# centreborelli/sat-bundleadjust

Measured on AMD Instinct MI355X. Metric: LM iters/sec at 200 cams x 1M pts x 10M obs (affine, R+T), higher is better.
Workload: dtype f64; 1 GPU; C4: 200 cams x 1000000 pts x 9998866 obs, affine, correction R+T, 1 fixed camera, seed 1; obs_per_rank0=9998866

## Files before the change

sat-bundleadjust_amd/csrc/satba_capi.hip:

```cpp
#include <hip/hip_runtime.h>

#include <algorithm>
#include <atomic>
#include <chrono>
#include <cmath>
#include <cstdarg>
#include <cstdio>
#include <cstdlib>
#include <cstring>
#include <new>
#include <string>
#include <thread>
#include <vector>

#include "../../include/satba.h"
#include "satba_chol.h"
#include "satba_kernels.h"
#include "satba_layout.h"
#include "satba_lm.h"
#include "satba_lmdev.h"
#include "satba_outliers.h"
#include "satba_triangulate.h"
#include "satba_rpcfit.h"
#include "satba_schur.h"
// ... 50 lines not shown
    long long K = 0, n_total = 0;
    int n_c = 0, n = 0, hdr = 0;
    int loss = 0;
    int camc_lds = 0, rpc_lds = 0;
    int cam_sums_lds = 1;
    int lin_rep_shift = 0;
    int deterministic = 0;
    double *d_fx = nullptr, *d_bbox = nullptr, *d_fxcost = nullptr, *d_fxcost_new = nullptr, *d_fxcost0 = nullptr;
    int *d_fxflag = nullptr, *d_fxe = nullptr;
    bool fxcost_valid = false, fxcost_new_valid = false, fxcost0_valid = false;
    bool decide_fused = false;
    double w_max = 1.0, n_max_cam = 1.0, fx_shrink = 1.0;
    int fx_fallbacks = 0;
    bool scales_by_tail = false;
    bool skip_lin_scales = false;
    const int* gate = nullptr;
    const double* Delta_dev = nullptr;
    const int* first_dev = nullptr;
    const double* coef_dev = nullptr;
    int fuse_prep = -1;
    bool prep_fused = false;
    const double* lam_force_dev = nullptr;
    const double* sub_args_dev = nullptr;
    struct LmDev* d_lm = nullptr;
    struct LmSummary* h_lm = nullptr;
    struct LmSummary* h_lm_dev = nullptr;
    long long lm_ticks_queued = 0;
    hipStream_t own_stream = nullptr;
    double f_scale = 1.0, lead = 1.0;
    hipStream_t stream = nullptr;
    Layout L;
    int unit_weights = 0;
    double *d_cam_static = nullptr, *d_rpc = nullptr;
    double *d_x = nullptr, *d_xnew = nullptr, *d_camc = nullptr, *d_camc_new = nullptr;
    double *d_scale_inv = nullptr, *d_g = nullptr, *d_gh = nullptr, *d_gn = nullptr, *d_q1 = nullptr, *d_wv = nullptr;
    double *d_U = nullptr, *d_gc = nullptr, *d_V = nullptr, *d_Vinv = nullptr, *d_PV = nullptr, *d_dc = nullptr, *d_dch = nullptr;
    double2 *d_f = nullptr, *d_ftmp = nullptr;
    bool f_valid = false;
    bool prof_lin = false;
    std::vector<hipEvent_t> prof_ev;
    size_t prof_used = 0;
    double* d_Jpm = nullptr;
    double *d_part = nullptr, *d_part3 = nullptr, *d_pair_part = nullptr;
    int2* d_items = nullptr;
    SchurItem* d_item_desc = nullptr;
    double2* d_W = nullptr;
    int2* d_items_w = nullptr;
    SchurItem* d_item_desc_w = nullptr;
    int n_item_blocks_w = 0;
    int2* d_items_merged = nullptr;
    SchurItem* d_item_desc_merged = nullptr;
    int n_item_blocks_merged = 0;
    int n_item_blocks = 0;
    int lin_grid = 0, cm_chunks = 1, cm_chunks_w = 1;
    double* d_red = nullptr;
    unsigned* d_red_cnt = nullptr;
    double* d_stage = nullptr;
    size_t stage_len = 0;
    int* d_fail = nullptr;
    double* d_dinv = nullptr;
    CholWork chol;
    bool scale_in_finish = false;
    bool s_scaled = false;
    double schur_lam = 0.0;
    const double* schur_lam_dev = nullptr;
    hipStream_t chol_stream = nullptr;
    hipEvent_t ev_fork = nullptr, ev_join = nullptr;
    int* d_arrive = nullptr;
    int* d_pair_cnt = nullptr;
    int* d_dg_cnt = nullptr;
    long long* d_ts = nullptr;
    int arrive_epoch = 0;
    bool decide2_fused = false;
    int msg_epoch = 0;
    double* msg_packed = nullptr;
    bool beside_last = false;
    bool beside_off = false;
    int beside_clean = 0;
    int beside_retry_after = 64;
    int beside_timeouts = 0;
    double* d_scal = nullptr;
    double* d_keep = nullptr;
    bool prepared = false;
    double *d_xb_own = nullptr, *d_xb = nullptr;
    long long xb_len = 0;
    double* h_pin = nullptr;
    bool dir_global = false;
    double* d_dir_tab = nullptr;
    void* h_stage = nullptr;
    size_t h_stage_len = 0;
    struct CopyLane { char* pin = nullptr; hipEvent_t ev[2] = {nullptr, nullptr}; };
    CopyLane lanes[8];
    hipStream_t copy_stream = nullptr;
    bool lanes_ready = false;
    double* d_err_keep = nullptr;
    hipEvent_t ev_err = nullptr;
    double* d_x0 = nullptr;
    bool linearized = false, have_step = false;
    double create_ms[8] = {0, 0, 0, 0, 0, 0, 0, 0};
    std::vector<void*> allocs;

    double* payload() const { return d_xb + hdr; }
    RedBuf red(int slot) const { return RedBuf{d_red + (size_t)slot * RED_MAX_NV * RED_MAX_GRID, d_red_cnt + slot}; }
};
enum { RB_RES = 0, RB_LIN = 1, RB_PREP = 2, RB_JVP = 3, RB_BS = 4, RB_SUB = 5, RB_TRIAL = 6, RB_MISC = 7 };

// ... 230 lines not shown
static int launch_linearize_kernel(satba_problem* p) {
    ObsArgs a = obs_args(p, false);
    a.sh = slice_split(p);
    a.rev = slice_rev(0);
    if (p->fuse_prep >= 0) {
        a.prep_scale = p->d_scale_inv; a.prep_gh = p->d_gh; a.prep_ghs = p->d_q1;
        a.prep_first = p->fuse_prep; a.prep_first_dev = p->first_dev;
    }
    const bool prof = p->prof_lin && p->prof_used + 2 <= 2 * 4096;
    if (prof) {
        while (p->prof_ev.size() < p->prof_used + 2) {
            hipEvent_t e;
            HIP_TRY(hipEventCreate(&e));
            p->prof_ev.push_back(e);
        }
        HIP_TRY(hipEventRecord(p->prof_ev[p->prof_used], p->stream));
    }
    SATBA_DISPATCH(p, TRY((launch_lin<MODEL, NP, CL, RL>(p, a))));
    if (prof) {
        HIP_TRY(hipEventRecord(p->prof_ev[p->prof_used + 1], p->stream));
        p->prof_used += 2;
    }
    return 0;
}

static int launch_cam_sums(satba_problem* p, double* U, double* gc) {
    ObsArgs a = obs_args(p, false);
    CamMajor cm = cam_major(p);
    SATBA_DISPATCH(p, hipLaunchKernelGGL((k_cam_sums<MODEL, NP>), dim3(p->M, p->cm_chunks), dim3(LINC_THREADS), 0, p->stream, a, cm, p->d_f, p->d_part3));
    HIP_TRY(hipGetLastError());
    const int total = p->M * cam_acc_len(p->NP);
    hipLaunchKernelGGL(k_cam_sums_finish, dim3((total + 255) / 256), dim3(256), 0, p->stream, p->M, p->NP, p->cm_chunks, p->d_part3, U, gc, p->gate);
    HIP_TRY(hipGetLastError());
    return 0;
}

static SchurArgs schur_args(const satba_problem* p) {
    SchurArgs s;
    s.PV = reinterpret_cast<const double2*>(p->d_PV);
    s.pair_ofs = p->L.pair_ofs; s.pair_pts = p->L.pair_pts; s.pair_pi = p->L.pair_pi; s.pair_pj = p->L.pair_pj;
    s.pair_ij = p->L.pair_ij; s.pair_part = p->d_pair_part; s.n_chunks = p->L.C; s.items = p->d_items; s.desc = p->d_item_desc;
    if (wmode(p) && p->L.wl_ready) {
        s.PV = p->d_W; s.wmode = 1; s.zero_fix = p->L.zero_fix; s.n_dg = p->L.n_dg;
        s.pair_rec = p->L.pair_rec; s.pair_kk = p->L.pair_kk; s.cm_rec = p->L.cm_rec; s.cm_sc = p->L.cm_sc; s.dg_part = p->d_part3;
        s.items = p->d_items_w; s.desc = p->d_item_desc_w;
    }
    return s;
}

template <int MODEL, int NP>
static int launch_schur(satba_problem* p, const ObsArgs& a, double* S, double* rhs) {
    CamMajor cm = cam_major(p);
    SchurArgs s = schur_args(p);
    const long long n_pairs = p->L.n_pairs;
    const bool pairs_run = n_pairs > 0 && p->L.E > 0;
    const bool dg_in_pairs = s.wmode && MODEL != RPC && pairs_run;
    int dchunks = (a.sc && MODEL != RPC) ? p->cm_chunks_w : p->cm_chunks;
    static const bool one_launch_env = !(getenv("SATBA_SCHUR_ONE_LAUNCH") && atoi(getenv("SATBA_SCHUR_ONE_LAUNCH")) == 0);
    const bool both = one_launch_env && !p->arrive_epoch && !dg_in_pairs && pairs_run;
    if (dg_in_pairs) dchunks = p->L.n_dg;
    else {
        if (s.wmode) cm.pt = p->L.cm_rec;
        s.diag_xcd = (dchunks % 8 == 0 && !getenv("SATBA_NO_DIAG_XCD")) ? 1 : 0;
        if (!both) hipLaunchKernelGGL((k_schur_diag<MODEL, NP>), dim3(p->M, dchunks), dim3(LINC_THREADS), 0, p->stream, a, cm, s, p->d_part3);
    }
    const int total = p->M * cam_acc_len(NP);
    const int nb_diag = (int)((std::max<long long>(8ll * total, p->hdr) + 255) / 256);
    auto finish = [&](int red_chunks, bool direct) {
        const long long outs = red_chunks > 1 ? n_pairs * NP * NP : 0;
        const bool scale = p->scale_in_finish && !direct && 1 + CH_MAX_STEPS <= nb_diag * 256;
        hipLaunchKernelGGL(k_schur_finish, dim3((unsigned)(nb_diag + (outs + 255) / 256)), dim3(256), 0, p->stream, p->M, NP, p->n_c, dchunks, p->d_part3,
                           p->schur_lam, p->schur_lam_dev, p->lead, p->d_gc, p->d_scale_inv, S, rhs, p->d_xb, (int)p->hdr, nb_diag, red_chunks,
                           p->L.pair_ij, p->d_pair_part, p->gate, scale ? p->d_dch : (double*)nullptr, scale ? p->d_fail : (int*)nullptr,
                           scale ? 1 + CH_MAX_STEPS : 0);
        p->s_scaled = scale;
    };
    if (p->arrive_epoch) {
        if (dg_in_pairs) {
            const int keep = dchunks;
            dchunks = 0;
            finish(1, true);
            dchunks = keep;
            s.dg_cnt = p->d_dg_cnt; s.dg_lam = p->schur_lam; s.dg_lam_dev = p->schur_lam_dev; s.dg_lead = p->lead; s.dg_gc = p->d_gc;
            s.dg_scale_inv = p->d_scale_inv; s.dg_rhs = rhs;
        } else finish(1, true);
        s.arrive = p->d_arrive; s.arrive_epoch = p->arrive_epoch; s.pair_cnt = p->d_pair_cnt; s.fail = p->d_fail;
    }
    int red_chunks = 1;
    if (n_pairs > 0 && p->L.E > 0) {
        const bool merged = a.unit && p->d_item_desc_merged;
        if (merged) { s.desc = p->d_item_desc_merged; s.items = p->d_items_merged; s.n_chunks = 1; }
        const dim3 igrid((unsigned)(merged ? p->n_item_blocks_merged : (s.wmode ? p->n_item_blocks_w : p->n_item_blocks)));
        if (both) {
            const int n_diag = p->M * dchunks, n_diag_pad = (n_diag + 7) & ~7;
            const dim3 bgrid(igrid.x + (unsigned)n_diag_pad);
            if (a.unit) hipLaunchKernelGGL((k_schur_both<MODEL, NP, true>), bgrid, dim3(256), 0, p->stream, a, cm, s, p->d_part3, S, n_diag, n_diag_pad, p->M, dchunks);
            else hipLaunchKernelGGL((k_schur_both<MODEL, NP, false>), bgrid, dim3(256), 0, p->stream, a, cm, s, p->d_part3, S, n_diag, n_diag_pad, p->M, dchunks);
        }
        else if (a.unit) hipLaunchKernelGGL((k_schur_pairs<MODEL, NP, true>), igrid, dim3(256), 0, p->stream, a, s, S);
        else hipLaunchKernelGGL((k_schur_pairs<MODEL, NP, false>), igrid, dim3(256), 0, p->stream, a, s, S);
        HIP_TRY(hipGetLastError());
        if (p->L.C > 1 && !merged) red_chunks = p->L.C;
        if (p->arrive_epoch && (a.unit ? red_chunks > 1 : false)) return fail(SATBA_E_STATE, "factorisation beside a unit-weight pair kernel with chunk partials");
    }
    if (!p->arrive_epoch) finish(red_chunks, n_pairs > 0 && p->L.E > 0 && red_chunks == 1);
    HIP_TRY(hipGetLastError());
    return 0;
}

static int launch_schur_kernel(satba_problem* p) {
    ObsArgs a = obs_args(p, false);
    double* S = p->payload();
    double* rhs = S + (size_t)p->n_c * p->n_c;
    SATBA_DISPATCH(p, TRY((launch_schur<MODEL, NP>(p, a, S, rhs))));
    return 0;
}

static int launch_backsub_kernel(satba_problem* p) {
    ObsArgs a = obs_args(p, false);
    a.sh = slice_split(p);
    a.rev = slice_rev(1);
    const int grid = slice_grid(p, BS_THREADS / 64, 2, a.sh);
    const size_t lds = p->model == AFFINE ? dir_table_bytes(p) : table_bytes(p);
    if (p->dir_global) {
        SATBA_DISPATCH(p, if constexpr (MODEL == AFFINE) {
            hipLaunchKernelGGL((k_affine_dir_tab<NP>), dim3(1), dim3(1024), 0, p->stream, a, p->d_dc, (const double*)nullptr, (const double*)nullptr);
            hipLaunchKernelGGL((k_backsub<MODEL, NP, CL, RL, true>), dim3(grid), dim3(BS_THREADS), 0, p->stream, a, p->d_dc, p->d_dch, p->lead,
                               p->d_Vinv, p->d_g, p->d_scale_inv, p->d_gh, p->d_gn, p->red(RB_BS), p->d_xb);
        });
    } else
    SATBA_DISPATCH(p, hipLaunchKernelGGL((k_backsub<MODEL, NP, CL, RL>), dim3(grid), dim3(BS_THREADS), lds, p->stream, a, p->d_dc, p->d_dch, p->lead,
                                         p->d_Vinv, p->d_g, p->d_scale_inv, p->d_gh, p->d_gn, p->red(RB_BS), p->d_xb));
    HIP_TRY(hipGetLastError());
    return 0;
}

static int launch_jvp(satba_problem* p, int nv, const double* q1, const double* q2, double* out, bool pre = false) {
    ObsArgs a = obs_args(p, false);
    a.sh = slice_split(p);
    a.rev = slice_rev(2);
    const int grid = slice_grid(p, JVP_THREADS / 64, 2, a.sh);
    const RedBuf rb = p->red(RB_JVP);
    if (p->dir_global && (nv == 2 || pre)) {
        SATBA_DISPATCH(p, if constexpr (MODEL == AFFINE) {
            hipLaunchKernelGGL((k_affine_dir_tab<NP>), dim3(1), dim3(1024), 0, p->stream, a, q1, nv == 2 ? q2 : nullptr, nv == 2 ? p->d_scale_inv : nullptr);
// ... 402 lines not shown
        TRY(dev_alloc(p, &p->d_cam_static, (size_t)p->M * p->c_p));
        if (p->model == RPC) TRY(dev_alloc(p, &p->d_rpc, (size_t)p->M * SATBA_RPC_TABLE_LEN));
        TRY(dev_alloc(p, &p->d_x, n)); TRY(dev_alloc(p, &p->d_xnew, n)); TRY(dev_alloc(p, &p->d_scale_inv, n));
        TRY(dev_alloc(p, &p->d_g, n)); TRY(dev_alloc(p, &p->d_gh, n)); TRY(dev_alloc(p, &p->d_gn, n));
        TRY(dev_alloc(p, &p->d_q1, n)); TRY(dev_alloc(p, &p->d_wv, n));
        TRY(dev_alloc(p, &p->d_camc, (size_t)p->M * CAMC)); TRY(dev_alloc(p, &p->d_camc_new, (size_t)p->M * CAMC));
        TRY(dev_alloc(p, &p->d_U, (size_t)p->M * p->NP * p->NP)); TRY(dev_alloc(p, &p->d_gc, p->n_c));
        TRY(dev_alloc(p, &p->d_V, (size_t)6 * p->N)); TRY(dev_alloc(p, &p->d_Vinv, (size_t)6 * p->N));
        TRY(dev_alloc(p, &p->d_PV, (size_t)PV_STRIDE * (p->N + 1)));
        HIP_TRY(hipMemset(p->d_PV + (size_t)PV_STRIDE * p->N, 0, sizeof(double) * PV_STRIDE));
        TRY(dev_alloc(p, &p->d_dc, p->n_c)); TRY(dev_alloc(p, &p->d_dch, p->n_c));
        const size_t Kz = (size_t)std::max<long long>(K, 1) + 64;
        TRY(dev_alloc(p, &p->d_f, Pz)); TRY(dev_alloc(p, &p->d_ftmp, Pz));
        if (p->model == RPC) TRY(dev_alloc(p, &p->d_Jpm, Kz * jrow_stride(p->NP)));
        TRY(dev_alloc(p, &p->d_fail, 1 + CH_MAX_STEPS));
        TRY(dev_alloc(p, &p->d_dinv, (size_t)((p->n_c + CH_NB - 1) / CH_NB) * CH_NB * CH_NB));
        {
            const size_t T = (size_t)(p->n_c + 63) / 64;
            TRY(dev_alloc(p, &p->chol.flags, T * T + 1)); TRY(dev_alloc(p, &p->chol.Linv, T * 4096 + 1)); TRY(dev_alloc(p, &p->chol.Cc, T * T * 64 + 1));
            TRY(dev_alloc(p, &p->chol.ctr, 4));
            HIP_TRY(hipMemset(p->chol.flags, 0, sizeof(int) * (T * T + 1)));
            HIP_TRY(hipMemset(p->chol.ctr, 0, sizeof(int) * 4));
        }
        TRY(dev_alloc(p, &p->d_scal, 8));
        TRY(dev_alloc(p, &p->d_fx, fx_scales_len(p->NP))); TRY(dev_alloc(p, &p->d_fxe, fx_exps_len(p->NP)));
        TRY(dev_alloc(p, &p->d_bbox, 6)); TRY(dev_alloc(p, &p->d_fxflag, 1));
        TRY(dev_alloc(p, &p->d_fxcost, 1)); TRY(dev_alloc(p, &p->d_fxcost_new, 1)); TRY(dev_alloc(p, &p->d_fxcost0, 1));
        HIP_TRY(hipMemset(p->d_bbox, 0, sizeof(double) * 6));
        HIP_TRY(hipMemset(p->d_fxflag, 0, sizeof(int)));
        if (const char* fs = getenv("SATBA_FX_SHRINK")) p->fx_shrink = atof(fs);
        TRY(dev_alloc(p, &p->d_lm, 1));
        HIP_TRY(hipMemset(p->d_lm, 0, sizeof(LmDev)));
        HIP_TRY(hipHostMalloc((void**)&p->h_lm, sizeof(LmSummary) + sizeof(LmDev), hipHostMallocMapped));
        memset(p->h_lm, 0, sizeof(LmSummary) + sizeof(LmDev));
        HIP_TRY(hipHostGetDevicePointer((void**)&p->h_lm_dev, p->h_lm, 0));
        TRY(dev_alloc(p, &p->d_keep, SATBA_KEEP_LEN));
        HIP_TRY(hipMemset(p->d_keep, 0, sizeof(double) * SATBA_KEEP_LEN));
        TRY(dev_alloc(p, &p->d_red, (size_t)RED_SLOTS * RED_MAX_NV * RED_MAX_GRID));
        TRY(dev_alloc(p, &p->d_red_cnt, RED_SLOTS));
        HIP_TRY(hipMemset(p->d_red_cnt, 0, sizeof(unsigned) * RED_SLOTS));
        p->lin_grid = lin_grid_for(p);
        TRY(dev_alloc(p, &p->d_part, (size_t)512 * p->M * cam_sum_len(p->NP)));
        {
            int chunks = 8;
            while (chunks < 64 && (long long)p->M * chunks < 512 && K / ((long long)p->M * (chunks + 8)) >= 4096) chunks += 8;
            while (chunks > 1 && K / ((long long)p->M * chunks) < 256) --chunks;
            int chunks_w = chunks;
            if (chunks >= 8) {
                chunks_w = std::min(64, 2 * chunks);
                while (chunks_w > chunks && K / ((long long)p->M * chunks_w) < 512) chunks_w -= 8;
            }
            if (const char* dc = getenv("SATBA_CM_CHUNKS")) chunks_w = chunks = std::max(1, std::min(256, atoi(dc)));
            p->cm_chunks = chunks; p->cm_chunks_w = chunks_w;
            TRY(dev_alloc(p, &p->d_part3, (size_t)p->M * std::max(64, std::max(chunks, chunks_w)) * (cam_acc_len(p->NP) + p->NP)));
        }
        if (p->L.C > 1) TRY(dev_alloc(p, &p->d_pair_part, (size_t)p->L.C * std::max<long long>(p->L.n_pairs, 1) * p->NP * p->NP));
        TRY(schur_item_table(p));
        p->stage_len = std::max<size_t>(std::max<size_t>(n, 2 * (size_t)K), (size_t)6 * p->N) + 16;
        TRY(dev_alloc(p, &p->d_stage, p->stage_len));
        p->xb_len = satba_exchange_len(p);
        TRY(dev_alloc(p, &p->d_xb_own, p->xb_len));
        p->d_xb = p->d_xb_own;
        HIP_TRY(hipHostMalloc((void**)&p->h_pin, sizeof(double) * (p->hdr + 64)));
        HIP_TRY(hipMemset(p->d_xb, 0, sizeof(double) * p->xb_len));
        HIP_TRY(hipMemset(p->d_scale_inv, 0, sizeof(double) * n));
        HIP_TRY(hipMemset(p->d_x, 0, sizeof(double) * n));
        HIP_TRY(hipMemset(p->d_xnew, 0, sizeof(double) * n));
        HIP_TRY(hipMemcpy(p->d_cam_static, d->cam_params, sizeof(double) * p->M * p->c_p, hipMemcpyHostToDevice));
        if (p->model == RPC)
            HIP_TRY(hipMemcpy(p->d_rpc, d->rpc_tables, sizeof(double) * p->M * SATBA_RPC_TABLE_LEN, hipMemcpyHostToDevice));
        return 0;
    }();
    if (rc) {
        satba_problem_destroy(p);
        return rc;
    }
    p->create_ms[4] = ms_since(t_create);
    *out = p;
    return 0;
}

void satba_problem_destroy(satba_problem* p) {
    if (!p) return;
    (void)hipSetDevice(p->device);
    (void)hipDeviceSynchronize();
#ifdef C3_STAMPS
    if (p->d_ts) {
        std::vector<long long> ts((size_t)20 * C3_TS);
        (void)hipMemcpy(ts.data(), p->d_ts, sizeof(long long) * ts.size(), hipMemcpyDeviceToHost);
        const int T = (p->n_c + 63) / 64;
        const long long t0 = ts[(size_t)T * C3_TS + 0];
        fprintf(stderr, "C3TS wait_begin 0 chain_start %.2f\n", (ts[(size_t)T * C3_TS + 1] - t0) * 0.01);
        for (int k = 0; k < T; ++k) {
            fprintf(stderr, "C3TS step %2d start %8.2f D_done %8.2f R %8.2f I %8.2f dnext %8.2f aux %8.2f nextD %8.2f | col arrived %8.2f handed %8.2f\n", k,
                    (ts[(size_t)k * C3_TS + 0] - t0) * 0.01, (ts[(size_t)k * C3_TS + 1] - t0) * 0.01, (ts[(size_t)k * C3_TS + 2] - t0) * 0.01,
                    (ts[(size_t)k * C3_TS + 3] - t0) * 0.01, (ts[(size_t)k * C3_TS + 4] - t0) * 0.01, (ts[(size_t)k * C3_TS + 5] - t0) * 0.01,
                    (ts[(size_t)k * C3_TS + 6] - t0) * 0.01, k >= 2 ? (ts[(size_t)T * C3_TS + k] - t0) * 0.01 : 0.0,
                    k >= 2 ? (ts[(size_t)(T + 1) * C3_TS + k] - t0) * 0.01 : 0.0);
        }
    }
#endif
    for (void* q : p->allocs) (void)hipFree(q);
    for (hipEvent_t e : p->prof_ev) (void)hipEventDestroy(e);
    if (p->h_pin) (void)hipHostFree(p->h_pin);
    if (p->h_stage) (void)hipHostFree(p->h_stage);
    for (auto& l : p->lanes) { if (l.pin) (void)hipHostFree(l.pin); for (hipEvent_t e : l.ev) if (e) (void)hipEventDestroy(e); }
    if (p->copy_stream) (void)hipStreamDestroy(p->copy_stream);
    if (p->ev_err) (void)hipEventDestroy(p->ev_err);
    if (p->h_lm) (void)hipHostFree(p->h_lm);
    if (p->own_stream) (void)hipStreamDestroy(p->own_stream);
    if (p->chol_stream) (void)hipStreamDestroy(p->chol_stream);
    if (p->ev_fork) (void)hipEventDestroy(p->ev_fork);
    if (p->ev_join) (void)hipEventDestroy(p->ev_join);
    delete p;
}

int satba_set_stream(satba_problem* p, void* hip_stream, int32_t use_own) {
    if (!p) return fail(SATBA_E_ARG, "null handle");
    HIP_TRY(hipSetDevice(p->device));
    HIP_TRY(hipStreamSynchronize(p->stream));
    p->stream = use_own ? p->own_stream : static_cast<hipStream_t>(hip_stream);
    return 0;
}

int64_t satba_header_len(const satba_problem* p) { return p ? p->hdr : 0; }

int64_t satba_exchange_len(const satba_problem* p) {
    if (!p) return 0;
    const long long lin = (long long)p->M * p->NP * p->NP + p->n_c;
    const long long sch = (long long)p->n_c * p->n_c + p->n_c;
    return p->hdr + (lin > sch ? lin : sch);
}

int satba_bind_exchange(satba_problem* p, double* device_ptr, int64_t len) {
    if (!p) return fail(SATBA_E_ARG, "null handle");
    if (!device_ptr) { p->d_xb = p->d_xb_own; return 0; }
    if (len < satba_exchange_len(p)) return fail(SATBA_E_ARG, "exchange buffer too small: %lld < %lld", (long long)len, (long long)satba_exchange_len(p));
    p->d_xb = device_ptr;
    return 0;
}

__global__ __launch_bounds__(256) void k_pack_lower(int n, int hdr, double* __restrict__ xb, double* __restrict__ packed, int unpack, int c_lo, int c_hi,
                                                    const int* gate) {
    SATBA_GATE(gate);
    const int j = blockIdx.x;
    if (j == n) {
        if (c_lo != 0) return;
        for (int i = threadIdx.x; i < hdr + n; i += 256) {
            double* a = i < hdr ? xb + i : xb + hdr + (size_t)n * n + (i - hdr);
            double* b = packed + i;
            if (unpack) __hip_atomic_store(a, __hip_atomic_load(b, __ATOMIC_RELAXED, __HIP_MEMORY_SCOPE_SYSTEM), __ATOMIC_RELAXED, __HIP_MEMORY_SCOPE_AGENT);
// ... 1289 lines not shown
```

sat-bundleadjust_amd/csrc/satba_schur.h:

```cpp
#pragma once
#include "satba_kernels.h"

namespace satba {

constexpr int PV_STRIDE = 16;
__device__ inline double schur_lambda(const double* __restrict__ hdr, double Delta, double lam_floor, double* __restrict__ keep, bool write) {
    const double gh_sq = hdr[1], jg_sq = hdr[2], xs_sq = hdr[3];
    if (!(Delta > 0.0)) {
        Delta = sqrt(xs_sq);
        if (Delta == 0.0) Delta = 1.0;
    }
    const double a = 0.5 * jg_sq, b = -gh_sq, ub = Delta / sqrt(gh_sq);
    double best = fmin(0.0, a * ub * ub + b * ub);
    if (a != 0.0) {
        const double ext = -0.5 * b / a;
        if (0.0 < ext && ext < ub) best = fmin(best, a * ext * ext + b * ext);
    }
    double lam = -best / (Delta * Delta);
    if (!(lam >= lam_floor)) lam = lam_floor;
    if (write) {
        keep[1] = fmax(keep[1], hdr[4]);
        keep[2] = gh_sq; keep[3] = jg_sq; keep[4] = xs_sq;
        keep[5] = lam;
        keep[6] = Delta;
// ... 63 lines not shown
#pragma unroll
        for (int k = 0; k < 8; ++k) {
            const int g = 64 * k + lane, r = g >> 3, q = g & 7;
            const double2 v = t[9 * r + (q < 6 ? q : 0)];
            const int at = w_fix[min(p0 + r, N - 1)];
            if (q < 6 && r < n_here) out[(size_t)at + q] = v;
        }
        return;
    }
    {
        double2* out = reinterpret_cast<double2*>(PV + PV_STRIDE * (size_t)p0);
#pragma unroll
        for (int k = 0; k < 8; ++k) {
            const int g = 64 * k + lane, r = g >> 3, q = g & 7;
            const double2 v = t[9 * r + (q < 6 ? q : 0)];
            if (q < 6 && r < n_here) out[g] = v;
        }
    }
}

struct SchurItem {
    long long lo, hi;
    int i, j;
    int pair, chunk;
};
struct SchurArgs {
    const double2* __restrict__ PV;
    const long long* __restrict__ pair_ofs;
    const int* __restrict__ pair_pts;
    const int* __restrict__ pair_pi;
    const int* __restrict__ pair_pj;
    const int2* __restrict__ pair_ij;
    double* __restrict__ pair_part;
    const int2* __restrict__ items;
    const struct SchurItem* __restrict__ desc;
    int n_chunks;
    int diag_xcd = 0;
    int wmode = 0, zero_fix = 0, n_dg = 1;
    const int* __restrict__ pair_rec = nullptr;
    const int* __restrict__ pair_kk = nullptr;
    const int* __restrict__ cm_rec = nullptr;
    const int* __restrict__ cm_sc = nullptr;
    double* __restrict__ dg_part = nullptr;
    int* dg_cnt = nullptr;
    double dg_lam = 0.0, dg_lead = 1.0;
    const double* dg_lam_dev = nullptr;
    const double* __restrict__ dg_gc = nullptr;
    const double* __restrict__ dg_scale_inv = nullptr;
    double* __restrict__ dg_rhs = nullptr;
    int* arrive = nullptr;
    int arrive_epoch = 0;
    int* pair_cnt = nullptr;
    int* fail = nullptr;
};
constexpr int SCHUR_ARRIVE_STRIDE = 32;

template <int N>
__device__ inline double wave_reduce_scatter(const double (&v)[N], int lane, int mask) {
    if constexpr (N == 1) {
        double t = v[0];
        for (int m = mask; m > 0; m >>= 1) t += __shfl_xor(t, m);
        return t;
    } else {
        constexpr int H = N / 2;
        const bool upper = (lane & mask) != 0;
        double w[H];
#pragma unroll
        for (int k = 0; k < H; ++k) {
            const double keep = upper ? v[k + H] : v[k];
            const double send = upper ? v[k] : v[k + H];
            w[k] = keep + __shfl_xor(send, mask);
        }
        return wave_reduce_scatter<H>(w, lane, mask >> 1);
    }
}
template <int N>
__device__ inline int rs_index(int lane) {
    int idx = 0, mask = 32;
    for (int h = N / 2; h >= 1; h >>= 1, mask >>= 1)
        if (lane & mask) idx += h;
    return idx;
}

__global__ void k_schur_item_desc(long long n_items, const int2* __restrict__ items, const int2* __restrict__ pair_ij,
                                  const long long* __restrict__ pair_ofs, int n_chunks, SchurItem* __restrict__ desc,
                                  const int* __restrict__ dg_ofs = nullptr, int n_dg = 1) {
    const long long e = (long long)blockIdx.x * blockDim.x + threadIdx.x;
    if (e >= n_items) return;
    const int2 it = items[e];
    SchurItem d;
    if (it.x == -1) { d.lo = d.hi = 0; d.i = d.j = -1; d.pair = -1; d.chunk = 0; }
    else if (it.x < -1) {
        const int cam = -2 - it.x;
        d.lo = dg_ofs[(size_t)cam * n_dg + it.y];
        d.hi = dg_ofs[(size_t)cam * n_dg + it.y + 1];
        d.i = d.j = cam; d.pair = -1; d.chunk = it.y;
    } else {
        const int2 ij = pair_ij[it.x];
        const int c0 = it.y < 0 ? 0 : it.y, c1 = it.y < 0 ? n_chunks : it.y + 1;
        d.lo = pair_ofs[(long long)it.x * (n_chunks + 1) + c0];
        d.hi = pair_ofs[(long long)it.x * (n_chunks + 1) + c1];
        d.i = ij.x; d.j = ij.y; d.pair = it.x; d.chunk = c0;
    }
    desc[e] = d;
}

__device__ __forceinline__ void schur_pair_publish(double* mine, size_t stride, int n_chunks, int chunk, int* cnt, int* arrive_row, int* fail,
                                                double* s_out, double total, bool writer) {
// ... 466 lines not shown
                __builtin_amdgcn_sched_barrier(0);
                compute(r_cur, pi_cur, pj_cur, si_cur, sj_cur, ti.v, tj.v);
                __builtin_amdgcn_sched_barrier(0);
                p_nxt = p_nn; c_cur = c_nxt;
                if constexpr (JROWS) { ji_cur = ji_nxt; jj_cur = jj_nxt; }
                pi_cur = pi_nxt; pj_cur = pj_nxt; pi_nxt = pi_nn; pj_nxt = pj_nn;
                idx += 64;
            }
        }
    }

    constexpr int NB2 = NP * NP;
    if constexpr (NB2 > 64) {
        schur_pairs_epilogue_wide<NP, UNITW>(a, s, S, bidx, lane, i, j, chunk, pair, n_pairs, acc);
        return;
    }
    constexpr int NPAD = NB2 <= 16 ? 16 : (NB2 <= 32 ? 32 : 64);
    static_assert(NB2 <= NPAD || NB2 > 64, "pair block reduction");
    double flat[NPAD];
#pragma unroll
    for (int e = 0; e < NPAD; ++e) flat[e] = (e < NB2) ? acc[e / NP][e % NP] : 0.0;
    const double cam_mask = (i < a.n_cam_fix || j < a.n_cam_fix) ? 0.0 : 1.0;
    const double total = cam_mask * wave_reduce_scatter<NPAD>(flat, lane, 32);
    const int e = rs_index<NPAD>(lane);
    const bool writer = (lane & (64 / NPAD - 1)) == 0 && e < NB2;
    int e_ = e, i_ = i, j_ = j, chunk_ = chunk;
    long long pair_ = pair;
    asm volatile("" : "+v"(e_), "+s"(i_), "+s"(j_), "+s"(chunk_), "+s"(pair_));
    if (s.arrive && bidx == 0 && threadIdx.x == 0)
        __hip_atomic_store(s.arrive + (size_t)SCHUR_ARRIVE_STRIDE * a.M, s.arrive_epoch, __ATOMIC_RELAXED, __HIP_MEMORY_SCOPE_AGENT);
    double* const s_out = S + (size_t)(j_ * NP + e_ % NP) + (size_t)(i_ * NP + e_ / NP) * a.n_c;
    if constexpr (!UNITW) {
        if (s.arrive && s.n_chunks > 1) {
            schur_pair_publish(s.pair_part + ((size_t)chunk_ * n_pairs + pair_) * NB2 + e_, (size_t)n_pairs * NB2, s.n_chunks, chunk_, s.pair_cnt + pair_,
                               s.arrive + (size_t)SCHUR_ARRIVE_STRIDE * i_, s.fail, s_out, total, writer);
            return;
        }
    }
    if (writer) {
        if (s.n_chunks > 1) s.pair_part[((size_t)chunk_ * n_pairs + pair_) * NB2 + e_] = total;
        else if (!s.arrive) *s_out = total;
        else __hip_atomic_store(s_out, total, __ATOMIC_RELAXED, __HIP_MEMORY_SCOPE_AGENT);
    }
    if (s.arrive && s.n_chunks == 1) {
        asm volatile("s_waitcnt vmcnt(0)" ::: "memory");
        if (lane == 0) __hip_atomic_fetch_add(s.arrive + (size_t)SCHUR_ARRIVE_STRIDE * i_, 1, __ATOMIC_RELAXED, __HIP_MEMORY_SCOPE_AGENT);
    }
}
template <int MODEL, int NP, bool UNITW>
__global__ __launch_bounds__(256) SATBA_PAIRS_WAVES_ATTR(MODEL, NP, UNITW) void k_schur_pairs(ObsArgs a, SchurArgs s, double* __restrict__ S) {
    SATBA_GATE(a.gate);
    __shared__ double2 s_coop[4 * 64 * 7];
    __shared__ unsigned s_idx[4][3 * 64];
    schur_pairs_body<MODEL, NP, UNITW>(a, s, S, blockIdx.x, s_coop, s_idx);
}


template <int MODEL, int NP, int THREADS>
__device__ __forceinline__ void schur_diag_walk(const ObsArgs& a, const double2* __restrict__ base, const int* __restrict__ lst_rec,
                                                const int* __restrict__ lst_sc, int rmul, int zero_rec, int cam, int lo, int hi, int tid,
                                                double2* my, double (&acc)[cam_acc_len(NP)]) {
    const double* cc = a.camc + (size_t)cam * CAMC;
    struct Rec { double2 r0, r1, r2, r3, r4, r5; };
    const int lane = tid & 63;
    int rsrc[6];
    const double2* psrc[6];
    double2* wdst[6];
#pragma unroll
    for (int t = 0; t < 6; ++t) {
        const int g = 64 * t + lane;
        rsrc[t] = g / 6; psrc[t] = base + g % 6; wdst[t] = my + (g / 6) * 7 + g % 6;
    }
    struct Coop { double2 c0, c1, c2, c3, c4, c5; };
    auto coop_load = [&](int p) {
        Coop o;
        o.c0 = psrc[0][(size_t)__shfl(p, rsrc[0])];
        o.c1 = psrc[1][(size_t)__shfl(p, rsrc[1])];
        o.c2 = psrc[2][(size_t)__shfl(p, rsrc[2])];
        o.c3 = psrc[3][(size_t)__shfl(p, rsrc[3])];
        o.c4 = psrc[4][(size_t)__shfl(p, rsrc[4])];
        o.c5 = psrc[5][(size_t)__shfl(p, rsrc[5])];
        return o;
    };
    const double2* mine = my + lane * 7;
    auto transpose = [&](const Coop& o) {
        Rec r;
        asm volatile("" ::: "memory");
        *wdst[0] = o.c0; *wdst[1] = o.c1; *wdst[2] = o.c2; *wdst[3] = o.c3; *wdst[4] = o.c4; *wdst[5] = o.c5;
        asm volatile("" ::: "memory");
        __builtin_amdgcn_wave_barrier();
        r.r0 = mine[0]; r.r1 = mine[1]; r.r2 = mine[2]; r.r3 = mine[3]; r.r4 = mine[4]; r.r5 = mine[5];
        asm volatile("" ::: "memory");
        __builtin_amdgcn_wave_barrier();
        return r;
    };
    constexpr bool AFAC = MODEL == AFFINE && NP <= 5;
    double Pm[2][3], Au[3] = {0.0, 0.0, 0.0}, tr[6] = {0.0, 0.0, 0.0, 0.0, 0.0, 0.0};
    if constexpr (AFAC) {
        const double fx = cc[CAMX + 2], fy = cc[CAMX + 3], sk = cc[CAMX + 4];
        Au[0] = fx; Au[1] = sk; Au[2] = fy;
#pragma unroll
        for (int k = 0; k < 3; ++k) { Pm[0][k] = fx * cc[6 + k] + sk * cc[9 + k]; Pm[1][k] = fy * cc[9 + k]; }
#pragma unroll
        for (int k = 0; k < 6; ++k) tr[k] = cc[k];
    }
    const int n_it = (hi - lo + THREADS - 1) / THREADS;
    if (n_it > 0) {
// ... 98 lines not shown
                for (int r = 0; r < NP; ++r) {
                    const double y0 = m00 * Jc[0][r] + m01 * Jc[1][r];
                    const double y1 = m01 * Jc[0][r] + m11 * Jc[1][r];
#pragma unroll
                    for (int q = r; q < NP; ++q) {
                        acc[k] -= Jc[0][q] * y0 + Jc[1][q] * y1;
                        acc[k] += ux * Jc[0][r] * Jc[0][q] + uy * Jc[1][r] * Jc[1][q];
                        ++k;
                    }
                }
#pragma unroll
                for (int r = 0; r < NP; ++r) acc[k++] -= Jc[0][r] * ag0 + Jc[1][r] * ag1;
            }
            __builtin_amdgcn_sched_barrier(0);
        }
    }
}

template <int MODEL, int NP>
__device__ __forceinline__ void schur_diag_body(const ObsArgs& a, const CamMajor& c, const SchurArgs& s, double* __restrict__ part, const int L, const int M,
                                                const int n_chunks, double2* s_coop, double (*s_red)[cam_acc_len(NP)]) {
    constexpr int CU = cam_acc_len(NP);
    int cam = L % M, chunk = L / M;
    if (s.diag_xcd) {
        const int x = L & 7, q = L >> 3;
        cam = q % M; chunk = (q / M) * 8 + x;
    }
    const int b = c.cam_ofs[cam], e = c.cam_ofs[cam + 1];
    const long long len = e - b;
    const int lo = b + (int)(len * chunk / n_chunks), hi = b + (int)(len * (chunk + 1) / n_chunks);
    const int lane = threadIdx.x & 63, wave = threadIdx.x >> 6;
    double acc[CU];
#pragma unroll
    for (int k = 0; k < CU; ++k) acc[k] = 0.0;
    schur_diag_walk<MODEL, NP, LINC_THREADS>(a, s.PV, c.pt, c.io, s.wmode ? 1 : PV_STRIDE / 2, s.wmode ? s.zero_fix : (PV_STRIDE / 2) * a.N, cam, lo, hi,
                                             (int)threadIdx.x, s_coop + wave * (64 * 7), acc);
    if (cam < a.n_cam_fix) {
#pragma unroll
        for (int k = 0; k < CU; ++k) acc[k] = 0.0;
    }
#pragma unroll
    for (int k = 0; k < CU; ++k) {
        const double t = wave_sum(acc[k]);
        if (lane == 0) s_red[wave][k] = t;
    }
    __syncthreads();
    if (threadIdx.x < CU) {
        double t = 0.0;
        for (int wv = 0; wv < LINC_THREADS / 64; ++wv) t += s_red[wv][threadIdx.x];
        part[((size_t)cam * n_chunks + chunk) * CU + threadIdx.x] = t;
    }
}
template <int MODEL, int NP>
__global__ __launch_bounds__(LINC_THREADS) void k_schur_diag(ObsArgs a, CamMajor c, SchurArgs s, double* __restrict__ part) {
    SATBA_GATE(a.gate);
    __shared__ double2 s_coop[(LINC_THREADS / 64) * 64 * 7];
    __shared__ double s_red[LINC_THREADS / 64][cam_acc_len(NP)];
    schur_diag_body<MODEL, NP>(a, c, s, part, (int)(blockIdx.y * gridDim.x + blockIdx.x), (int)gridDim.x, (int)gridDim.y, s_coop, s_red);
}
static_assert(LINC_THREADS == 256, "k_schur_both: both bodies run 256 threads");
template <int MODEL, int NP, bool UNITW>
__global__ __launch_bounds__(256) SATBA_PAIRS_WAVES_ATTR(MODEL, NP, UNITW) void k_schur_both(ObsArgs a, CamMajor c, SchurArgs s, double* __restrict__ part, double* __restrict__ S,
                                                                                      int n_diag, int n_diag_pad, int M, int n_chunks) {
    SATBA_GATE(a.gate);
    __shared__ double2 s_coop[4 * 64 * 7];
    __shared__ unsigned s_idx[4][3 * 64];
    __shared__ double s_red[4][cam_acc_len(NP)];
    if ((int)blockIdx.x < n_diag_pad) {
        if ((int)blockIdx.x < n_diag) schur_diag_body<MODEL, NP>(a, c, s, part, (int)blockIdx.x, M, n_chunks, s_coop, s_red);
        return;
    }
    schur_pairs_body<MODEL, NP, UNITW>(a, s, S, blockIdx.x - (unsigned)n_diag_pad, s_coop, s_idx);
}

__global__ __launch_bounds__(256) void k_schur_finish(int M, int NP, int n_c, int n_chunks, const double* __restrict__ part, double lam,
                                                      const double* __restrict__ lam_dev, double lead, const double* __restrict__ gc,
                                                      const double* __restrict__ scale_inv, double* __restrict__ S, double* __restrict__ rhs,
                                                      double* __restrict__ xb, int hdr_len, int nb_diag, int red_chunks,
                                                      const int2* __restrict__ pair_ij, const double* __restrict__ pair_part, const int* gate,
                                                      double* __restrict__ rhs_scaled = nullptr, int* __restrict__ clear = nullptr, int n_clear = 0) {
    SATBA_GATE(gate);
    if ((int)blockIdx.x >= nb_diag) {
        const long long n_pairs = (long long)M * (M - 1) / 2;
        const int NB2 = NP * NP;
        const long long idx = (long long)(blockIdx.x - nb_diag) * blockDim.x + threadIdx.x;
        if (idx >= n_pairs * NB2) return;
        const long long pair = idx / NB2;
        const int e = (int)(idx % NB2);
        double t = 0.0;
        int ch = 0;
        for (; ch + 4 <= red_chunks; ch += 4) {
            const double p0 = pair_part[((size_t)ch * n_pairs + pair) * NB2 + e], p1 = pair_part[((size_t)(ch + 1) * n_pairs + pair) * NB2 + e];
            const double p2 = pair_part[((size_t)(ch + 2) * n_pairs + pair) * NB2 + e], p3 = pair_part[((size_t)(ch + 3) * n_pairs + pair) * NB2 + e];
            t += p0; t += p1; t += p2; t += p3;
        }
        for (; ch < red_chunks; ++ch) t += pair_part[((size_t)ch * n_pairs + pair) * NB2 + e];
        const int2 ij = pair_ij[pair];
        const int r = e / NP, q = e % NP;
        if (rhs_scaled) t /= scale_inv[ij.y * NP + q] * scale_inv[ij.x * NP + r];
        S[(size_t)(ij.y * NP + q) + (size_t)(ij.x * NP + r) * n_c] = t;
        return;
    }
    if (lam_dev) lam = *lam_dev;
    const int CU = cam_acc_len(NP);
    const int gid = blockIdx.x * blockDim.x + threadIdx.x, idx = gid >> 3, sub = gid & 7;
    if (gid < hdr_len) xb[gid] = 0.0;
    if (gid < n_clear) clear[gid] = 0;
    if (n_chunks <= 0) return;
    const bool live = idx < M * CU;
    const int cam = live ? idx / CU : 0, k = live ? idx % CU : 0;
    const double t = schur_diag_total<false>(part, cam, n_chunks, CU, k, sub, live);
    if (!live || sub != 0) return;
// ... 5 lines not shown
```

Measured before the change: 908.1 LM iters/sec.

## Add diag Schur kernel with 192-thread camera units replacing one-launch path

Adds k_schur_diag_units, which assigns each camera chunk to a unit of one or three waves (64 or 192 threads) instead of a full 256-thread block. It optionally interleaves chunks across XCDs. For unit-weight, non-RPC, L2-loss problems with enough camera chunks, the default now uses 192-thread units. That default disables the fused k_schur_both launch, so the diag and pairs kernels run as separate launches. Also adds compile-time-gated per-workgroup timestamp instrumentation, which is off by default.

```diff
diff --git a/sat-bundleadjust_amd/csrc/satba_capi.hip b/sat-bundleadjust_amd/csrc/satba_capi.hip
--- a/sat-bundleadjust_amd/csrc/satba_capi.hip
+++ b/sat-bundleadjust_amd/csrc/satba_capi.hip
@@ -126,6 +126,11 @@
     SchurItem* d_item_desc_merged = nullptr;
     int n_item_blocks_merged = 0;
     int n_item_blocks = 0;
+#ifdef SATBA_SCHUR_STAMPS
+    long long* d_sst = nullptr;
+    unsigned sst_pairs = 0, sst_diag = 0;
+#endif
+    int diag_unit = 256, diag_interleave = 0;
     int lin_grid = 0, cm_chunks = 1, cm_chunks_w = 1;
     double* d_red = nullptr;
     unsigned* d_red_cnt = nullptr;
@@ -462,17 +467,37 @@
 static int launch_schur(satba_problem* p, const ObsArgs& a, double* S, double* rhs) {
     CamMajor cm = cam_major(p);
     SchurArgs s = schur_args(p);
+#ifdef SATBA_SCHUR_STAMPS
+    s.stamps = p->d_sst;
+#endif
     const long long n_pairs = p->L.n_pairs;
     const bool pairs_run = n_pairs > 0 && p->L.E > 0;
     const bool dg_in_pairs = s.wmode && MODEL != RPC && pairs_run;
     int dchunks = (a.sc && MODEL != RPC) ? p->cm_chunks_w : p->cm_chunks;
-    static const bool one_launch_env = !(getenv("SATBA_SCHUR_ONE_LAUNCH") && atoi(getenv("SATBA_SCHUR_ONE_LAUNCH")) == 0);
-    const bool both = one_launch_env && !p->arrive_epoch && !dg_in_pairs && pairs_run;
+    const char* ol = getenv("SATBA_SCHUR_ONE_LAUNCH");
+    const bool one_launch_env = !(ol && atoi(ol) == 0);
+    const bool both = one_launch_env && !p->arrive_epoch && !dg_in_pairs && pairs_run && p->diag_unit == 256;
     if (dg_in_pairs) dchunks = p->L.n_dg;
     else {
         if (s.wmode) cm.pt = p->L.cm_rec;
         s.diag_xcd = (dchunks % 8 == 0 && !getenv("SATBA_NO_DIAG_XCD")) ? 1 : 0;
-        if (!both) hipLaunchKernelGGL((k_schur_diag<MODEL, NP>), dim3(p->M, dchunks), dim3(LINC_THREADS), 0, p->stream, a, cm, s, p->d_part3);
+        if (p->diag_unit != 256) {
+            if (s.diag_xcd && p->diag_interleave) s.diag_xcd = 2;
+#ifdef SATBA_SCHUR_STAMPS
+            p->sst_diag = (unsigned)((p->M + 256 / p->diag_unit - 1) / (256 / p->diag_unit) * dchunks);
+#endif
+#define SATBA_DIAG_UNITS(UT)                                                                                                                         \
+    hipLaunchKernelGGL((k_schur_diag_units<MODEL, NP, UT>), dim3((unsigned)((p->M + DiagUnit<UT>::UPW - 1) / DiagUnit<UT>::UPW * dchunks)),       \
+                       dim3(DiagUnit<UT>::THREADS), 0, p->stream, a, cm, s, p->d_part3, p->M, dchunks)
+            if (p->diag_unit == 64) SATBA_DIAG_UNITS(64);
+            else SATBA_DIAG_UNITS(192);
+#undef SATBA_DIAG_UNITS
+        } else if (!both) {
+            hipLaunchKernelGGL((k_schur_diag<MODEL, NP>), dim3(p->M, dchunks), dim3(LINC_THREADS), 0, p->stream, a, cm, s, p->d_part3);
+#ifdef SATBA_SCHUR_STAMPS
+            p->sst_diag = (unsigned)(p->M * dchunks);
+#endif
+        }
     }
     const int total = p->M * cam_acc_len(NP);
     const int nb_diag = (int)((std::max<long long>(8ll * total, p->hdr) + 255) / 256);
@@ -501,6 +526,9 @@
         const bool merged = a.unit && p->d_item_desc_merged;
         if (merged) { s.desc = p->d_item_desc_merged; s.items = p->d_items_merged; s.n_chunks = 1; }
         const dim3 igrid((unsigned)(merged ? p->n_item_blocks_merged : (s.wmode ? p->n_item_blocks_w : p->n_item_blocks)));
+#ifdef SATBA_SCHUR_STAMPS
+        p->sst_pairs = both ? 0u : igrid.x;
+#endif
         if (both) {
             const int n_diag = p->M * dchunks, n_diag_pad = (n_diag + 7) & ~7;
             const dim3 bgrid(igrid.x + (unsigned)n_diag_pad);
@@ -1009,9 +1037,20 @@
             }
             if (const char* dc = getenv("SATBA_CM_CHUNKS")) chunks_w = chunks = std::max(1, std::min(256, atoi(dc)));
             p->cm_chunks = chunks; p->cm_chunks_w = chunks_w;
+            if (p->model != RPC && p->loss == 0 && p->unit_weights && (long long)p->M * chunks > 8 * 96) p->diag_unit = 192;
+            if (const char* du = getenv("SATBA_DIAG_UNIT")) {
+                const int u = atoi(du);
+                if (u != 64 && u != 192 && u != 256) return fail(SATBA_E_ARG, "SATBA_DIAG_UNIT: 64, 192 or 256");
+                p->diag_unit = u;
+            }
+            p->diag_interleave = getenv("SATBA_DIAG_INTERLEAVE") && atoi(getenv("SATBA_DIAG_INTERLEAVE")) != 0;
             TRY(dev_alloc(p, &p->d_part3, (size_t)p->M * std::max(64, std::max(chunks, chunks_w)) * (cam_acc_len(p->NP) + p->NP)));
         }
         if (p->L.C > 1) TRY(dev_alloc(p, &p->d_pair_part, (size_t)p->L.C * std::max<long long>(p->L.n_pairs, 1) * p->NP * p->NP));
+#ifdef SATBA_SCHUR_STAMPS
+        TRY(dev_alloc(p, &p->d_sst, (size_t)4 * SCHUR_STAMP_WGS));
+        HIP_TRY(hipMemset(p->d_sst, 0, sizeof(long long) * 4 * SCHUR_STAMP_WGS));
+#endif
         TRY(schur_item_table(p));
         p->stage_len = std::max<size_t>(std::max<size_t>(n, 2 * (size_t)K), (size_t)6 * p->N) + 16;
         TRY(dev_alloc(p, &p->d_stage, p->stage_len));
@@ -1054,6 +1093,22 @@
                     (ts[(size_t)k * C3_TS + 3] - t0) * 0.01, (ts[(size_t)k * C3_TS + 4] - t0) * 0.01, (ts[(size_t)k * C3_TS + 5] - t0) * 0.01,
                     (ts[(size_t)k * C3_TS + 6] - t0) * 0.01, k >= 2 ? (ts[(size_t)T * C3_TS + k] - t0) * 0.01 : 0.0,
                     k >= 2 ? (ts[(size_t)(T + 1) * C3_TS + k] - t0) * 0.01 : 0.0);
+        }
+    }
+#endif
+#ifdef SATBA_SCHUR_STAMPS
+    if (p->d_sst && getenv("SATBA_SCHUR_STAMPS_OUT")) {
+        if (FILE* fo = fopen(getenv("SATBA_SCHUR_STAMPS_OUT"), "w")) {
+            std::vector<long long> st((size_t)4 * SCHUR_STAMP_WGS);
+            (void)hipMemcpy(st.data(), p->d_sst, sizeof(long long) * st.size(), hipMemcpyDeviceToHost);
+            for (int k = 0; k < 2; ++k) {
+                const unsigned n = std::min<unsigned>(k ? p->sst_diag : p->sst_pairs, SCHUR_STAMP_WGS);
+                for (unsigned w = 0; w < n; ++w) {
+                    const long long t0 = st[2 * ((size_t)k * SCHUR_STAMP_WGS + w)], v = st[2 * ((size_t)k * SCHUR_STAMP_WGS + w) + 1];
+                    if (t0) fprintf(fo, "%s %u %lld %lld %lld\n", k ? "diag" : "pairs", w, t0, v >> 16, v & 0xffff);
+                }
+            }
+            fclose(fo);
         }
     }
 #endif
diff --git a/sat-bundleadjust_amd/csrc/satba_schur.h b/sat-bundleadjust_amd/csrc/satba_schur.h
--- a/sat-bundleadjust_amd/csrc/satba_schur.h
+++ b/sat-bundleadjust_amd/csrc/satba_schur.h
@@ -139,8 +139,30 @@
     int arrive_epoch = 0;
     int* pair_cnt = nullptr;
     int* fail = nullptr;
+#ifdef SATBA_SCHUR_STAMPS
+    long long* stamps = nullptr;
+#endif
 };
 constexpr int SCHUR_ARRIVE_STRIDE = 32;
+#ifdef SATBA_SCHUR_STAMPS
+constexpr int SCHUR_STAMP_WGS = 32768;
+#define SATBA_STAMP_BEGIN() const long long stamp_t0_ = wall_clock64()
+#define SATBA_DIAG_STAMP_OCC __attribute__((amdgpu_waves_per_eu(3)))
+#define SATBA_STAMP_END(st, wg) schur_stamp((st), (wg), stamp_t0_)
+__device__ __forceinline__ void schur_stamp(long long* st, unsigned wg, long long t0) {
+    __syncthreads();
+    if (st && threadIdx.x == 0 && wg < (unsigned)SCHUR_STAMP_WGS) {
+        longlong2 v;
+        v.x = t0;
+        v.y = ((wall_clock64() - t0) << 16) | (long long)(__smid() & 0xffffu);
+        *reinterpret_cast<longlong2*>(st + 2 * (size_t)wg) = v;
+    }
+}
+#else
+#define SATBA_STAMP_BEGIN() do {} while (0)
+#define SATBA_DIAG_STAMP_OCC
+#define SATBA_STAMP_END(st, wg) do {} while (0)
+#endif
 
 template <int N>
 __device__ inline double wave_reduce_scatter(const double (&v)[N], int lane, int mask) {
@@ -713,7 +735,9 @@
     SATBA_GATE(a.gate);
     __shared__ double2 s_coop[4 * 64 * 7];
     __shared__ unsigned s_idx[4][3 * 64];
+    SATBA_STAMP_BEGIN();
     schur_pairs_body<MODEL, NP, UNITW>(a, s, S, blockIdx.x, s_coop, s_idx);
+    SATBA_STAMP_END(s.stamps, blockIdx.x);
 }
 
 
@@ -918,12 +942,68 @@
     }
 }
 template <int MODEL, int NP>
-__global__ __launch_bounds__(LINC_THREADS) void k_schur_diag(ObsArgs a, CamMajor c, SchurArgs s, double* __restrict__ part) {
+__global__ __launch_bounds__(LINC_THREADS) SATBA_DIAG_STAMP_OCC void k_schur_diag(ObsArgs a, CamMajor c, SchurArgs s, double* __restrict__ part) {
     SATBA_GATE(a.gate);
     __shared__ double2 s_coop[(LINC_THREADS / 64) * 64 * 7];
     __shared__ double s_red[LINC_THREADS / 64][cam_acc_len(NP)];
+    SATBA_STAMP_BEGIN();
     schur_diag_body<MODEL, NP>(a, c, s, part, (int)(blockIdx.y * gridDim.x + blockIdx.x), (int)gridDim.x, (int)gridDim.y, s_coop, s_red);
-}
+    SATBA_STAMP_END(s.stamps ? s.stamps + 2 * SCHUR_STAMP_WGS : nullptr, blockIdx.y * gridDim.x + blockIdx.x);
+}
+template <int UT>
+struct DiagUnit {
+    static_assert(UT == 64 || UT == 192, "unit of one or three waves");
+    static constexpr int THREADS = UT == 192 ? 192 : 256, UPW = THREADS / UT, WPU = UT / 64;
+};
+template <int MODEL, int NP, int UT>
+__global__ __launch_bounds__(DiagUnit<UT>::THREADS) SATBA_DIAG_STAMP_OCC void k_schur_diag_units(ObsArgs a, CamMajor c, SchurArgs s, double* __restrict__ part, int M, int n_chunks) {
+    SATBA_GATE(a.gate);
+    constexpr int CU = cam_acc_len(NP), BT = DiagUnit<UT>::THREADS, UPW = DiagUnit<UT>::UPW, WPU = DiagUnit<UT>::WPU;
+    __shared__ double2 s_coop[(BT / 64) * 64 * 7];
+    __shared__ double s_red[BT / 64][CU];
+    SATBA_STAMP_BEGIN();
+    const int L = (int)blockIdx.x, Mg = (M + UPW - 1) / UPW;
+    int grp = L % Mg, chunk = L / Mg;
+    if (s.diag_xcd) {
+        const int x = L & 7, q = L >> 3, nrep = n_chunks >> 3;
+        if (s.diag_xcd == 2) { grp = q / nrep; chunk = (q % nrep) * 8 + x; }
+        else { grp = q % Mg; chunk = (q / Mg) * 8 + x; }
+    }
+    const int lane = threadIdx.x & 63, wave = threadIdx.x >> 6, unit = wave / WPU;
+    const int cam_u = grp * UPW + unit;
+    const bool live = cam_u < M;
+    const int cam = __builtin_amdgcn_readfirstlane(live ? cam_u : M - 1);
+    int lo = 0, hi = 0;
+    if (live) {
+        const int b = c.cam_ofs[cam], e = c.cam_ofs[cam + 1];
+        const long long len = e - b;
+        lo = b + (int)(len * chunk / n_chunks); hi = b + (int)(len * (chunk + 1) / n_chunks);
+    }
+    double acc[CU];
+#pragma unroll
+    for (int k = 0; k < CU; ++k) acc[k] = 0.0;
+    schur_diag_walk<MODEL, NP, UT>(a, s.PV, c.pt, c.io, s.wmode ? 1 : PV_STRIDE / 2, s.wmode ? s.zero_fix : (PV_STRIDE / 2) * a.N, cam, lo, hi,
+                                   (int)threadIdx.x - unit * UT, s_coop + wave * (64 * 7), acc);
+    if (cam < a.n_cam_fix) {
+#pragma unroll
+        for (int k = 0; k < CU; ++k) acc[k] = 0.0;
+    }
+#pragma unroll
+    for (int k = 0; k < CU; ++k) {
+        const double t = wave_sum(acc[k]);
+        if (lane == 0) s_red[wave][k] = t;
+    }
+    __syncthreads();
+    for (int o = threadIdx.x; o < UPW * CU; o += BT) {
+        const int u = o / CU, k = o % CU, cam_o = grp * UPW + u;
+        if (cam_o >= M) continue;
+        double t = 0.0;
+        for (int wv = 0; wv < WPU; ++wv) t += s_red[u * WPU + wv][k];
+        part[((size_t)cam_o * n_chunks + chunk) * CU + k] = t;
+    }
+    SATBA_STAMP_END(s.stamps ? s.stamps + 2 * SCHUR_STAMP_WGS : nullptr, blockIdx.x);
+}
+
 static_assert(LINC_THREADS == 256, "k_schur_both: both bodies run 256 threads");
 template <int MODEL, int NP, bool UNITW>
 __global__ __launch_bounds__(256) SATBA_PAIRS_WAVES_ATTR(MODEL, NP, UNITW) void k_schur_both(ObsArgs a, CamMajor c, SchurArgs s, double* __restrict__ part, double* __restrict__ S,
```

After: 912.6 LM iters/sec, median of 6. Within noise of the previous version (+0.5%).
